# edwinyosorahardjo/compressjs-flattened

Measured on AMD Instinct MI355X. Metric: bzip2 -9 compress MB/s at 1/2/4/8 MI355X; bit-exact output size vs ref, higher is better.
Workload: dtype u32; 1 GPU; Bzip2.compressFile level 9 (899981-byte blocks) on 1 x 100000000 bytes enwik8-shaped synthetic text (tools/textgen.c seed 1), device-resident; per_gpu_bytes=100000000, level=9, parallelism=1 GPU

## Files before the change

### compressjs-flattened_amd/csrc/bwt.hip

```cpp
#include "radix.hpp"
#include <stdlib.h>
#include <string.h>
#include <type_traits>

namespace cjs {

struct Geom { uint32_t nb, stride, n_last; };
__device__ __forceinline__ uint32_t blk_len(const Geom& g, uint32_t blk) { return blk == g.nb - 1 ? g.n_last : g.stride; }
struct VarGeom { uint32_t nb, stride, n_last; const uint32_t* len; };
__device__ __forceinline__ uint32_t blk_len(const VarGeom& g, uint32_t blk) { return g.len[blk]; }

template <typename G>
__global__ __launch_bounds__(256) void bwt_init_keys(const uint8_t* __restrict__ T, G g, int cyclic, int nsym, uint32_t M,
                                                     uint64_t* __restrict__ key, uint32_t* __restrict__ val) {
  for (uint64_t a = (uint64_t)blockIdx.x * 256 + threadIdx.x; a < M; a += (uint64_t)gridDim.x * 256) {
    const uint32_t blk = (uint32_t)(a / g.stride), i = (uint32_t)(a - (uint64_t)blk * g.stride), n = blk_len(g, blk);
    const uint8_t* t = T + (size_t)blk * g.stride;
    uint64_t k = 0;
    if constexpr (std::is_same_v<G, VarGeom>) {
      uint32_t x = i;
      if (i >= n) k = (1ull << (8 * nsym)) | i;
      else for (int j = 0; j < nsym; j++) { k = (k << 8) | t[x]; if (++x == n) x = 0; }
      k |= (uint64_t)blk << (8 * nsym + 1);
    } else if (cyclic) {
// ... 57 lines not shown
    k[it] = key[base + (loc < nvalid ? loc : nvalid - 1u)] >> gshift;
  }
  if (threadIdx.x == 0) sk[0] = base ? key[base - 1] >> gshift : 0;
  if (threadIdx.x == 64) sk[RS_TILE + 1] = base + RS_TILE < A ? key[base + RS_TILE] >> gshift : 0;
#pragma unroll
  for (int it = 0; it < 16; it++) sk[1u + (uint32_t)it * 256 + threadIdx.x] = k[it];
  __syncthreads();
#pragma unroll
  for (int it = 0; it < 16; it++) {
    const uint32_t loc = (uint32_t)it * 256 + threadIdx.x;
    const uint64_t a = base + loc;
    if (loc < nvalid) {
      const bool nh = a == 0 || a == bnd || sk[loc] != k[it];
      const bool nx = a + 1 == A || a + 1 == bnd || sk[loc + 2] != k[it];
      const bool single = nh && nx;
      surv += !single;
      heads += nh && !single;
      if (nh) last = (uint32_t)a + 1u;
    }
    const uint64_t hb = __ballot(loc < nvalid && (base + loc == 0 || base + loc == bnd || sk[loc] != k[it]));
    if (lane_id() == 0) hword[it * 4 + wave_id()] = hb != 0;
  }
  __syncthreads();
  if (threadIdx.x < 8 && base + (threadIdx.x + 1u) * 512u <= A) {
    uint32_t any = 0;
    for (int j = 0; j < 8; j++) any |= hword[threadIdx.x * 8 + j];
    if (!any) atomicOr(big_flag, 1u);
  }
  surv = block_sum<256>(surv, sm);
  heads = block_sum<256>(heads, sm);
  last = wave_max(last);
  if (lane_id() == 0) sm[wave_id()] = last;
  __syncthreads();
  if (threadIdx.x == 0) {
    uint32_t m = sm[0]; for (int i = 1; i < 4; i++) m = sm[i] > m ? sm[i] : m;
    tile_cnt[blockIdx.x] = surv; tile_cnt[T + blockIdx.x] = heads; tile_cnt[2 * (size_t)T + blockIdx.x] = m;
  }
}

constexpr uint32_t HF_NEW = 1u, HF_OLD = 2u;
__device__ __forceinline__ uint32_t hf_bits16(const uint4& v, int bit) {
  const uint32_t M = 0x01020408u;
  const uint32_t n0 = (((v.x >> bit) & 0x01010101u) * M) >> 24, n1 = (((v.y >> bit) & 0x01010101u) * M) >> 24;
  const uint32_t n2 = (((v.z >> bit) & 0x01010101u) * M) >> 24, n3 = (((v.w >> bit) & 0x01010101u) * M) >> 24;
  return (n0 & 15u) | ((n1 & 15u) << 4) | ((n2 & 15u) << 8) | ((n3 & 15u) << 12);
}
__device__ __forceinline__ uint4 hf_load16(const uint8_t* __restrict__ hflag, uint64_t base, uint32_t nvalid, int tid, uint32_t& valid) {
  const uint32_t first = (uint32_t)tid * 16u;
  const uint32_t nv = nvalid > first ? (nvalid - first < 16u ? nvalid - first : 16u) : 0u;
  valid = (1u << nv) - 1u;
  uint4 v = make_uint4(0u, 0u, 0u, 0u);
  if (nv) v = *reinterpret_cast<const uint4*>(hflag + base + first);
  return v;
}
__global__ __launch_bounds__(256) void bwt_key_flags(const uint64_t* __restrict__ key, uint32_t A, uint8_t* __restrict__ hflag) {
  for (uint64_t a = (uint64_t)blockIdx.x * 256 + threadIdx.x; a < A; a += (uint64_t)gridDim.x * 256) {
    const uint64_t k = key[a], p = a ? key[a - 1] : ~k;
    hflag[a] = (uint8_t)((k != p ? HF_NEW : 0u) | ((k >> 20) != (p >> 20) ? HF_OLD : 0u));
  }
}
__global__ __launch_bounds__(256) void bwt_flags_bytes(const uint8_t* __restrict__ hflag, uint32_t A, uint32_t* __restrict__ tile_cnt, uint32_t T,
                                                       uint32_t* __restrict__ big_flag) {
  __shared__ uint32_t nhs[257];
  __shared__ uint32_t sm[4];
  const int tid = threadIdx.x;
  const uint64_t base = (uint64_t)blockIdx.x * RS_TILE;
  const uint32_t nvalid = (uint32_t)((uint64_t)A - base < RS_TILE ? (uint64_t)A - base : RS_TILE);
  uint32_t valid;
  const uint4 v = hf_load16(hflag, base, nvalid, tid, valid);
  const uint32_t nh = hf_bits16(v, 0) & valid;
  nhs[tid] = nh | (~valid & 0xFFFFu);
  if (tid == 0) nhs[256] = base + RS_TILE < A ? (uint32_t)hflag[base + RS_TILE] & HF_NEW : 1u;
  __syncthreads();
  const uint32_t nx = ((nhs[tid] >> 1) | (nhs[tid + 1] << 15)) & 0xFFFFu;
  const uint32_t single = nh & nx;
  uint32_t surv = (uint32_t)__popc(valid & ~single), heads = (uint32_t)__popc(nh & ~single);
  uint32_t last = nh ? (uint32_t)base + (uint32_t)tid * 16u + 32u - (uint32_t)__clz(nh) : 0u;
  {
    const uint64_t any = __ballot(nh != 0);
    const uint32_t run0 = (uint32_t)wave_id() * 2u;
    if (lane_id() == 0) {
      bool bad = false;
      for (uint32_t b = 0; b < 2; b++) bad |= base + (uint64_t)(run0 + b + 1u) * 512u <= A && (uint32_t)(any >> (32 * b)) == 0u;
      if (bad) atomicOr(big_flag, 1u);
    }
  }
  surv = block_sum<256>(surv, sm);
  heads = block_sum<256>(heads, sm);
  last = wave_max(last);
  if (lane_id() == 0) sm[wave_id()] = last;
  __syncthreads();
  if (tid == 0) {
    uint32_t m = sm[0]; for (int i = 1; i < 4; i++) m = sm[i] > m ? sm[i] : m;
    tile_cnt[blockIdx.x] = surv; tile_cnt[T + blockIdx.x] = heads; tile_cnt[2 * (size_t)T + blockIdx.x] = m;
  }
}

__global__ __launch_bounds__(1024) void bwt_scan_tiles(uint32_t* __restrict__ tile_cnt, uint32_t T, uint32_t* __restrict__ counters,
                                                      uint32_t* __restrict__ host_mirror ) {
  __shared__ uint32_t sm[16];
  __shared__ uint32_t mx[1024];
  uint32_t c0 = 0, c1 = 0, cm = 0;
  for (uint32_t base = 0; base < T; base += 1024) {
    const uint32_t i = base + threadIdx.x;
    const bool ok = i < T;
    uint32_t t0, t1;
    const uint32_t v0 = ok ? tile_cnt[i] : 0u, v1 = ok ? tile_cnt[T + i] : 0u, v2 = ok ? tile_cnt[2 * (size_t)T + i] : 0u;
    const uint32_t e0 = block_excl_sum<1024>(v0, sm, t0);
    const uint32_t e1 = block_excl_sum<1024>(v1, sm, t1);
    const uint32_t im = block_incl_max<1024>(v2, sm);
    mx[threadIdx.x] = im;
    __syncthreads();
    const uint32_t prev = threadIdx.x ? mx[threadIdx.x - 1] : 0u;
    const uint32_t chunk_max = mx[1023];
    __syncthreads();
    if (ok) {
      tile_cnt[i] = c0 + e0; tile_cnt[T + i] = c1 + e1;
      tile_cnt[2 * (size_t)T + i] = prev > cm ? prev : cm;
    }
    c0 += t0; c1 += t1; cm = chunk_max > cm ? chunk_max : cm;
  }
  if (threadIdx.x == 0) { counters[0] = c0; counters[1] = c1; host_mirror[0] = c0; host_mirror[1] = c1; host_mirror[4] = counters[4]; counters[4] = 0; }
}

__device__ __forceinline__ uint64_t class_head_before(const uint64_t* __restrict__ key, uint64_t seg0, uint64_t base, int shift, int lane) {
  if (base == seg0) return base;
  const uint64_t target = key[base] >> shift;
  const uint64_t off = base - seg0;
  const uint32_t back = off < 64u ? (uint32_t)off : 64u;
  const bool eq = (uint32_t)lane < back && (key[base - 1u - (uint32_t)lane] >> shift) == target;
  const uint64_t ne = ~__ballot(eq);
  const uint32_t m = ne ? (uint32_t)__builtin_ctzll(ne) : 64u;
  if (m < 64u || off <= 64u) return base - m;
  uint64_t lo = seg0, hi = base - 64u;
  while (hi > lo) {
    const uint64_t len = hi - lo, step = (len + 63u) / 64u, idx = lo + (uint64_t)lane * step;
    const bool hit = idx >= hi || (key[idx] >> shift) == target;
    const uint64_t hits = __ballot(hit);
    const uint32_t j = hits ? (uint32_t)__builtin_ctzll(hits) : 64u;
    if (!j) { hi = lo; break; }
    const uint64_t nhi = lo + (uint64_t)j * step;
    lo += (uint64_t)(j - 1u) * step + 1u;
    if (j < 64u && nhi < hi) hi = nhi;
  }
  return hi;
// ... 81 lines not shown
    const uint32_t first = (uint32_t)lane * 64u;
    const uint32_t nv = nvalid > first ? (nvalid - first < 64u ? nvalid - first : 64u) : 0u;
    const uint64_t vm = nv == 64 ? ~0ull : ((1ull << nv) - 1ull);
    uint64_t ms;
    if constexpr (FIRST) ms = m_sg[lane];
    else {
      const uint64_t mhx = mh | ~vm;
      uint32_t nb = __shfl_down((uint32_t)(mhx & 1ull), 1, 64);
      if (lane == 63) nb = nx_s;
      ms = mh & ((mhx >> 1) | ((uint64_t)nb << 63));
      m_sg[lane] = ms;
    }
    const uint32_t sv = (uint32_t)__popcll(vm & ~ms), hd = (uint32_t)__popcll(mh & ~ms);
    const uint32_t lastrel = mh ? first + 63u - (uint32_t)__builtin_clzll(mh) + 1u : 0u;
    const uint32_t is = wave_incl_sum(sv), ih = wave_incl_sum(hd), im = wave_incl_max(lastrel);
    uint32_t em = __shfl_up(im, 1, 64);
    if (lane == 0) em = 0;
    wp_s[lane] = is - sv; wp_h[lane] = ih - hd; wp_head[lane] = em;
    if (SWEEP == 1 && lane == 63) {
      tile_cnt[tile] = is; tile_cnt[T + tile] = ih; tile_cnt[2 * (size_t)T + tile] = im ? (uint32_t)base + im : 0u;
    }
    if (SWEEP == 1) {
      const uint64_t nz = __ballot(mh != 0);
      bool bad = false;
#pragma unroll
      for (int b = 0; b < 8; b++) bad |= base + (uint64_t)(b + 1) * 512u <= A && ((nz >> (8 * b)) & 0xFFull) == 0;
      if (bad && lane == 0) atomicOr(big_flag, 1u);
    }
  }
  __syncthreads();
  if (SWEEP == 1) carry = carry_s;
  const uint64_t lt = (1ull << lane) - 1ull, le = lane == 63 ? ~0ull : ((2ull << lane) - 1ull);
  uint32_t ub[16];
#pragma unroll
  for (int it = 0; it < 16; it++) ub[it] = 0u;
  const bool emits = U != nullptr && SWEEP != 1;
  if (emits && !carried) {
#pragma unroll
    for (int it = 0; it < 16; it++) {
      const uint32_t e = (uint32_t)it * 256u + tid;
      const bool sing = e < nvalid && ((m_sg[it * 4 + w] >> lane) & 1ull);
      const uint32_t p = FIRST ? (uint32_t)(base + e) : p16[FIRST ? 0 : it];
      const uint32_t vv = (PACKED ? (uint32_t)sk[e + 1] : v16[PACKED ? 0 : it]) & PK_POS_MASK;
      const uint32_t blk = p / g.stride;
      ub[it] = sing ? (uint32_t)Tx[(size_t)blk * g.stride + (vv ? vv - 1u : blk_len(g, blk) - 1u)] : 0u;
    }
  }
#pragma unroll
  for (int it = 0; it < 16; it++) {
    const uint32_t e = (uint32_t)it * 256u + tid;
// ... 14 lines not shown
      }
      const uint32_t p = FIRST ? (uint32_t)a : p16[FIRST ? 0 : it];
      const uint32_t vraw = PACKED ? (uint32_t)sk[e + 1] : v16[PACKED ? 0 : it];
      const uint32_t vv = vraw & PK_POS_MASK;
      const uint32_t pb = PACKED ? (vraw >> PK2_PREV_SHIFT) & 0xFFu : vraw >> VAL_PREV_SHIFT;
      const uint32_t blk = p / g.stride;
      const uint32_t head_pos = p - ((uint32_t)a - head_a);
      if (!keeps_rank && (SWEEP == 0 || (uint32_t)(vv >= hsplit) == half)) R[(size_t)blk * g.stride + vv] = head_pos - blk * g.stride;
      if (SWEEP == 1) continue;
      if ((ms >> lane) & 1ull) {
        if (U) U[p] = (uint8_t)(carried ? pb : ub[it]);
        else __builtin_nontemporal_store(vv, SA + p);
      } else {
        const uint32_t so = sbase + wp_s[wi] + (uint32_t)__popcll(~ms & lt);
        const uint32_t ho = hbase + wp_h[wi] + (uint32_t)__popcll(mh & ~ms & le);
        __builtin_nontemporal_store(carried ? (vv | (pb << VAL_PREV_SHIFT)) : vv, nval + so); __builtin_nontemporal_store(p, npos + so); __builtin_nontemporal_store(ho - 1u, ngord + so);
      }
    }
  }
}

constexpr uint32_t TS_WIN = 4096, TS_MAXGRP = 1024, TS_NOM = TS_WIN - TS_MAXGRP, TS_TINY = 64, TS_GT = 2048;

template <typename G> struct TsGatherT { const uint32_t* R; const uint32_t* pos; const uint32_t* gord; uint32_t h; int cyclic; G g; };
template <bool WMAP> __device__ __forceinline__ uint32_t ts_slot(int s, int tid) {
  return WMAP ? (uint32_t)(tid >> 6) * 1024u + (uint32_t)s * 64u + (uint32_t)(tid & 63) : (uint32_t)s * 256u + (uint32_t)tid;
}
template <bool WMAP, typename TG>
__device__ __forceinline__ uint32_t ts_fused_load(const TG& tg, const uint32_t* __restrict__ val, uint64_t wb, uint32_t L,
                                                  uint32_t (&go)[16], uint32_t (&pv)[16], uint32_t (&pp)[16], uint32_t& gprev) {
  const int tid = threadIdx.x;
#pragma unroll
  for (int s = 0; s < 16; s++) { const uint32_t x = ts_slot<WMAP>(s, tid); go[s] = tg.gord[wb + (x < L ? x : L - 1u)]; }
#pragma unroll
  for (int s = 0; s < 16; s++) { const uint32_t x = ts_slot<WMAP>(s, tid); pv[s] = val[wb + (x < L ? x : L - 1u)]; }
#pragma unroll
  for (int s = 0; s < 16; s++) { const uint32_t x = ts_slot<WMAP>(s, tid); pp[s] = tg.pos[wb + (x < L ? x : L - 1u)]; }
  uint32_t li = 0;
  gprev = 0xFFFFFFFFu;
  if (wb) {
    const uint32_t* q = tg.gord + wb - TS_MAXGRP + (uint32_t)tid * 4u;
    const uint32_t q0 = q[0], q1 = q[1], q2 = q[2], q3 = q[3], g0 = tg.gord[wb];
    gprev = tg.gord[wb - 1];
    li = q3 != g0 ? (uint32_t)tid * 4u + 4u : q2 != g0 ? (uint32_t)tid * 4u + 3u : q1 != g0 ? (uint32_t)tid * 4u + 2u : q0 != g0 ? (uint32_t)tid * 4u + 1u : 0u;
  }
#pragma unroll
// ... 12 lines not shown
__device__ __forceinline__ void ts_fused_gather(const TG& tg, uint32_t need, const uint32_t (&pv)[16], uint32_t (&pp)[16], uint32_t (&rk20)[16]) {
  uint32_t past = 0;
#pragma unroll
  for (int s = 0; s < 16; s++) {
    const uint32_t blk = pp[s] / tg.g.stride, n = blk_len(tg.g, blk);
    uint32_t j = (pv[s] & PK_POS_MASK) + tg.h;
    if (tg.cyclic) { if (j >= n) j %= n; }
    else if (j >= n) { j = 0; past |= 1u << s; }
    pp[s] = blk * tg.g.stride + j;
  }
#pragma unroll
  for (int s = 0; s < 16; s++) rk20[s] = tg.R[((need >> s) & 1u) ? pp[s] : pp[0]];
#pragma unroll
  for (int s = 0; s < 16; s++) rk20[s] = ((past >> s) & 1u) ? 0u : rk20[s] + 1u;
}

__device__ __forceinline__ void ts_ce(uint64_t& a, uint64_t& b, bool up) {
  const bool sw = (a > b) == up;
  const uint64_t x = sw ? b : a, y = sw ? a : b;
  a = x; b = y;
}
template <typename TG>
__global__ __launch_bounds__(256) void bwt_tile_sort(uint64_t* __restrict__ key, uint32_t* __restrict__ val, uint8_t* __restrict__ hflag, uint32_t A,
                                                     uint8_t* __restrict__ dflag, TG tg, uint32_t Tt) {
  __shared__ uint64_t sk[TS_WIN];
  __shared__ uint64_t hm[64];
  __shared__ int32_t wlast[64], wnext[64];
  uint32_t* gk = (uint32_t*)sk;
  const int tid = threadIdx.x, w = tid >> 6, lane = tid & 63;
  __shared__ uint32_t lired[4];
  const uint32_t win = xcd_tile(blockIdx.x, Tt);
  if (win >= Tt) return;
  const uint64_t wb = (uint64_t)win * TS_NOM;
  const uint64_t we = (wb + TS_WIN < A) ? wb + TS_WIN : A;
  const uint32_t L = (uint32_t)(we - wb);
  uint64_t r[16];
  uint32_t pv[16], go[16], pp[16];
  uint32_t gprev;
  {
    const uint32_t li = wave_max(ts_fused_load<false>(tg, val, wb, L, go, pv, pp, gprev));
    if (lane == 0) lired[w] = li;
  }
#pragma unroll
  for (int it = 0; it < 16; it++) gk[(uint32_t)it * 256u + tid] = go[it];
  __syncthreads();
#pragma unroll
  for (int it = 0; it < 16; it++) {
// ... 21 lines not shown
  __shared__ uint32_t mpre[65];
  int any_medium = 0;
  uint32_t hx16[16];
  uint32_t prev_end = 0, needm = 0;
  {
    const uint32_t a01 = lired[0] > lired[1] ? lired[0] : lired[1], a23 = lired[2] > lired[3] ? lired[2] : lired[3];
    prev_end = ts_prev_end(wb, L, we == A, a01 > a23 ? a01 : a23, hm, wnext);
  }
#pragma unroll
  for (int it = 0; it < 16; it++) {
    const uint32_t x = (uint32_t)it * 256u + tid;
    const int wi = it * 4 + w;
    const uint64_t m = hm[wi];
    const uint64_t le = lane == 63 ? ~0ull : ((2ull << lane) - 1ull);
    const uint64_t gt = lane == 63 ? 0ull : ~((2ull << lane) - 1ull);
    int hx = (m & le) ? wi * 64 + 63 - (int)__builtin_clzll(m & le) : wlast[wi];
    int nx = (m & gt) ? wi * 64 + (int)__builtin_ctzll(m & gt) : wnext[wi];
    if (nx > (int)L) nx = (we == A) ? (int)L : (int)TS_WIN + 1;
    const bool valid = x < L;
    const bool small = valid && hx >= 0 && nx <= (int)L && (uint32_t)(nx - hx) <= TS_MAXGRP;
    const bool owned = small && (uint32_t)hx < TS_NOM;
    const bool medium = owned && (nx - hx) > (int)TS_TINY;
    if (owned && dflag) dflag[wb + x] = 0;
    hx16[it] = owned ? ((uint32_t)hx | ((uint32_t)(nx - hx) << 16)) : 0xFFFFFFFFu;
    const uint64_t mb = __ballot(medium);
    if (lane == 0) mm[wi] = mb;
    any_medium |= medium ? 1 : 0;
    needm |= (valid && x >= prev_end && (owned || x < TS_NOM)) ? 1u << it : 0u;
  }
  {
    uint32_t rk20[16];
    ts_fused_gather(tg, needm, pv, pp, rk20);
#pragma unroll
    for (int it = 0; it < 16; it++) {
      const uint32_t x = (uint32_t)it * 256u + tid;
      const bool owned = hx16[it] != 0xFFFFFFFFu;
      if (((needm >> it) & 1u) && !owned) key[wb + x] = ((uint64_t)go[it] << 20) | rk20[it];
      r[it] = owned ? (((uint64_t)(hx16[it] & 0xFFFFu) << 52) | ((uint64_t)rk20[it] << 32) | pv[it])
                    : (((uint64_t)x << 52) | (0xFFFFFull << 32));
    }
  }
  __syncthreads();
  uint32_t* sk32 = reinterpret_cast<uint32_t*>(sk);
#pragma unroll
  for (int it = 0; it < 16; it++) { const uint32_t x = (uint32_t)it * 256u + tid; sk32[x] = ((uint32_t)(r[it] >> 32) << 12) | x; }
  any_medium = __syncthreads_or(any_medium);
// ... 57 lines not shown
      for (uint32_t t = tid; t < (P >> 2); t += 256) {
        const uint32_t i0 = ((t & ~(hj - 1)) << 2) | (t & (hj - 1));
        const bool up = (i0 & kk) == 0;
        uint64_t e0 = sk[i0], e1 = sk[i0 | hj], e2 = sk[i0 | j], e3 = sk[i0 | j | hj];
        ts_ce(e0, e2, up); ts_ce(e1, e3, up); ts_ce(e0, e1, up); ts_ce(e2, e3, up);
        sk[i0] = e0; sk[i0 | hj] = e1; sk[i0 | j] = e2; sk[i0 | j | hj] = e3;
      }
      __syncthreads();
    }
  }
#pragma unroll
  for (int it = 0; it < 16; it++) {
    if (cix[it] != 0xFFFFFFFFu) {
      const uint32_t x = (uint32_t)it * 256u + tid;
      const uint32_t c = cix[it];
      const uint64_t e = sk[c], pe = c ? sk[c - 1] : ~e;
      hflag[wb + x] = (uint8_t)(((e >> 32) != (pe >> 32) ? HF_NEW : 0u) | ((e >> 52) != (pe >> 52) ? HF_OLD : 0u));
      val[wb + x] = (uint32_t)e;
    }
  }
}
template <typename TG>
__global__ __launch_bounds__(256) void bwt_tile_sort_radix(uint64_t* __restrict__ key, uint32_t* __restrict__ val, uint8_t* __restrict__ hflag, uint32_t A,
                                                           uint8_t* __restrict__ dflag, TG tg, uint32_t Tt) {
  __shared__ uint64_t se[TS_WIN];
  __shared__ uint64_t hm[64];
  __shared__ int32_t wlast[64], wnext[64];
  __shared__ uint32_t wcnt[4][256];
  __shared__ uint32_t sm[4];
  uint32_t* gk = (uint32_t*)se;
  const int tid = threadIdx.x, w = tid >> 6, lane = tid & 63;
  __shared__ uint32_t lired[4];
  const uint32_t win = xcd_tile(blockIdx.x, Tt);
  if (win >= Tt) return;
  const uint64_t wb = (uint64_t)win * TS_NOM;
  const uint64_t we = (wb + TS_WIN < A) ? wb + TS_WIN : A;
  const uint32_t L = (uint32_t)(we - wb);
  uint32_t rk20[16], go[16], pv[16], pp[16];
  uint32_t gprev;
  {
    const uint32_t li = wave_max(ts_fused_load<true>(tg, val, wb, L, go, pv, pp, gprev));
    if (lane == 0) lired[w] = li;
#pragma unroll
    for (int s = 0; s < 16; s++) gk[ts_slot<true>(s, tid)] = go[s];
  }
  __syncthreads();
#pragma unroll
// ... 15 lines not shown
    int ir = wave_incl_max(rv);
    int er = __shfl_up(ir, 1, 64); if (lane == 0) er = -((int)TS_WIN + 1);
    const int en = -__shfl(er, 63 - lane, 64);
    wlast[lane] = el; wnext[lane] = en;
  }
  __syncthreads();
  uint32_t prev_end = 0;
  {
    const uint32_t a01 = lired[0] > lired[1] ? lired[0] : lired[1], a23 = lired[2] > lired[3] ? lired[2] : lired[3];
    prev_end = ts_prev_end(wb, L, we == A, a01 > a23 ? a01 : a23, hm, wnext);
  }
  uint32_t comp[16];
  uint32_t ownm = 0, needm = 0;
#pragma unroll
  for (int s = 0; s < 16; s++) {
    const uint32_t x = (uint32_t)w * 1024u + (uint32_t)s * 64u + lane;
    const int wi = w * 16 + s;
    const uint64_t m = hm[wi];
    const uint64_t le = lane == 63 ? ~0ull : ((2ull << lane) - 1ull);
    const uint64_t gt = lane == 63 ? 0ull : ~((2ull << lane) - 1ull);
    const int hx = (m & le) ? wi * 64 + 63 - (int)__builtin_clzll(m & le) : wlast[wi];
    int nx = (m & gt) ? wi * 64 + (int)__builtin_ctzll(m & gt) : wnext[wi];
    if (nx > (int)L) nx = (we == A) ? (int)L : (int)TS_WIN + 1;
    const bool owned = x < L && hx >= 0 && nx <= (int)L && (uint32_t)(nx - hx) <= TS_MAXGRP && (uint32_t)hx < TS_NOM;
    if (owned && dflag) dflag[wb + x] = 0;
    ownm |= owned ? 1u << s : 0u;
    needm |= (x < L && x >= prev_end && (owned || x < TS_NOM)) ? 1u << s : 0u; comp[s] = (uint32_t)hx;
  }
  {
    ts_fused_gather(tg, needm, pv, pp, rk20);
#pragma unroll
    for (int s = 0; s < 16; s++) {
      const uint32_t x = (uint32_t)w * 1024u + (uint32_t)s * 64u + lane;
      const bool owned = (ownm >> s) & 1u;
      if (((needm >> s) & 1u) && !owned) key[wb + x] = ((uint64_t)go[s] << 20) | rk20[s];
      comp[s] = owned ? ((comp[s] << 20) | rk20[s]) : (x << 20);
    }
  }
#pragma unroll
  for (int s = 0; s < 16; s++) if (!((ownm >> s) & 1u)) pv[s] = 0u;
  if (!__syncthreads_or((int)ownm)) return;
#pragma unroll 1
  for (int shift = 0; shift < 32; shift += 8) {
    for (int i = tid; i < 1024; i += 256) (&wcnt[0][0])[i] = 0;
    __syncthreads();
    uint32_t rk[16];
#pragma unroll
    for (int s = 0; s < 16; s++) rk[s] = rank_step((comp[s] >> shift) & 255u, wcnt[w]);
// ... 5 lines not shown
      wcnt[0][tid] = ex; wcnt[1][tid] = ex + c0; wcnt[2][tid] = ex + c0 + c1; wcnt[3][tid] = ex + c0 + c1 + c2;
    }
    __syncthreads();
#pragma unroll
    for (int s = 0; s < 16; s++) {
      const uint32_t d = (comp[s] >> shift) & 255u;
      se[wcnt[w][d] + rk[s]] = ((uint64_t)comp[s] << 32) | pv[s];
    }
    __syncthreads();
#pragma unroll
    for (int s = 0; s < 16; s++) {
      const uint64_t e = se[(uint32_t)w * 1024u + (uint32_t)s * 64u + lane];
      comp[s] = (uint32_t)(e >> 32); pv[s] = (uint32_t)e;
    }
    __syncthreads();
  }
#pragma unroll
  for (int s = 0; s < 16; s++) {
    if ((ownm >> s) & 1u) {
      const uint32_t x = (uint32_t)w * 1024u + (uint32_t)s * 64u + lane;
      const uint32_t pc = x ? (uint32_t)(se[x - 1] >> 32) : ~comp[s];
      hflag[wb + x] = (uint8_t)((comp[s] != pc ? HF_NEW : 0u) | ((comp[s] >> 20) != (pc >> 20) ? HF_OLD : 0u));
      val[wb + x] = pv[s];
    }
  }
}
__global__ __launch_bounds__(1024) void scan_u32_single(uint32_t* __restrict__ arr, uint32_t n, uint32_t* __restrict__ total, uint32_t* __restrict__ host_total) {
  __shared__ uint32_t sm[16];
  uint32_t carry = 0;
  for (uint32_t base = 0; base < n; base += 1024) {
    const uint32_t i = base + threadIdx.x;
    uint32_t v = i < n ? arr[i] : 0u, tot;
    const uint32_t ex = block_excl_sum<1024>(v, sm, tot);
    if (i < n) arr[i] = carry + ex;
    carry += tot;
  }
  if (threadIdx.x == 0) { *total = carry; *host_total = carry; }
}
__device__ __forceinline__ void defer_flags(uint32_t A, const uint8_t* __restrict__ dflag, const uint64_t* __restrict__ key, uint64_t a0,
                                            uint32_t& f, uint32_t& heads, uint64_t (&k8)[8]) {
  f = 0; heads = 0;
  if (a0 >= A) return;
  if (a0 + 8 <= A) {
    const uint64_t w = *(const uint64_t*)(dflag + a0);
#pragma unroll
    for (int j = 0; j < 8; j++) f |= (uint32_t)((w >> (8 * j)) & 1ull) << j;
// ... 155 lines not shown
  for (uint32_t i = threadIdx.x; i < n; i += 256) cnt += r[i] == r0;
  cnt = block_sum<256>(cnt, sm);
  if (threadIdx.x == 0) pidx[blk] = r0 + cnt - 1u;
}

__global__ __launch_bounds__(256) void bwt_emit_sentinel(const uint8_t* __restrict__ T, Geom g, uint32_t M,
                                                         const uint32_t* __restrict__ SA, const uint32_t* __restrict__ R, uint8_t* __restrict__ U, uint32_t Tn) {
  const uint32_t tile = xcd_tile(blockIdx.x, Tn);
  if (tile >= Tn) return;
#pragma unroll 4
  for (int it = 0; it < 16; it++) {
    const uint64_t a = (uint64_t)tile * RS_TILE + (uint32_t)it * 256 + threadIdx.x;
    if (a >= M) break;
    const uint32_t blk = (uint32_t)(a / g.stride), p = (uint32_t)(a - (uint64_t)blk * g.stride), n = blk_len(g, blk);
    const uint8_t* t = T + (size_t)blk * g.stride;
    uint8_t* u = U + (size_t)blk * g.stride;
    const uint32_t s = __builtin_nontemporal_load(SA + a);
    const uint32_t p0 = R[(size_t)blk * g.stride];
    if (p == p0) u[0] = t[n - 1];
    else u[p < p0 ? p + 1 : p] = t[s - 1];
  }
}

enum Counter { CN_SURVIVORS = 0, CN_GROUPS = 1, CN_DEFERRED = 2, CN_DEFERRED_GROUPS = 3, CN_LARGE_GROUP = 4 };

size_t BwtWork::bytes_needed(size_t cap) {
  const size_t T = RadixWork::hist_tiles_for(cap);
  size_t b = 0;
  auto add = [&](size_t n) { b += (n + 255) & ~(size_t)255; };
  add(cap * 8); add(cap * 8); add(cap * 4); add(cap * 4); add(cap * 4); add(cap * 4); add(cap * 4);
  add(cap * 4); add(cap * 4); add(cap); add(cap);
  add(RadixWork::hist_words(T) * 4); add(256 * RadixWork::segs_for(cap) * 4); add(3 * T * 4); add(64);
  return b + 4096;
}
int BwtWork::carve(Arena& a, size_t cap_) {
  cap = cap_;
  const size_t T = RadixWork::hist_tiles_for(cap);
  key[0] = a.take<uint64_t>(cap); key[1] = a.take<uint64_t>(cap);
  val[0] = a.take<uint32_t>(cap); val[1] = a.take<uint32_t>(cap);
  pos[0] = a.take<uint32_t>(cap); pos[1] = a.take<uint32_t>(cap);
  gord = a.take<uint32_t>(cap);
  R = a.take<uint32_t>(cap); SA = a.take<uint32_t>(cap); dflag = a.take<uint8_t>(cap); hflag = a.take<uint8_t>(cap);
  CJS_TRY(rs.carve(a, T, RadixWork::segs_for(cap)));
  tile_cnt = a.take<uint32_t>(3 * T); counters = a.take<uint32_t>(16);
  if (!counters) return CJS_E_OUT_OF_MEMORY;
  if (!h_counters) CJS_HIP_TRY(hipHostMalloc((void**)h_counters.put(), 64));
  if (!ev_scan) CJS_HIP_TRY(hipEventCreateWithFlags(ev_scan.put(), hipEventDisableTiming));
  return 0;
}

struct Plan {
  bool segmented, packed;
  bool sweeps;
  int nsym, bits;
  int gs1, carried;
  SegGeom sg; GenSrc gen;
  const uint8_t* Tx; uint8_t* U;
};
template <typename G>
static Plan plan_round1(const BwtWork& w, const G& g, bool cyclic, const uint8_t* d_T, uint8_t* d_U) {
  constexpr bool VAR = std::is_same_v<G, VarGeom>;
  Plan p;
  const int sym_bits = cyclic ? 8 : 9;
  const uint32_t tps = ((g.nb > 1 ? g.stride : g.n_last) + RS_TILE - 1) / RS_TILE;
  p.segmented = !VAR && (uint64_t)g.nb * tps <= w.rs.hist_tiles && g.nb <= w.rs.bintot_segs && getenv("CJS_NO_SEGMENTED_SORT") == nullptr;
  p.packed = p.segmented && cyclic;
  p.sweeps = g.nb >= 8 && p.packed;
  const int blk_bits = bits_for(g.nb - 1) + (VAR ? 1 : 0);
  p.nsym = p.segmented || (64 - blk_bits) / sym_bits > 7 ? 7 : (64 - blk_bits) / sym_bits;
  p.bits = p.nsym * sym_bits + (p.segmented ? 0 : blk_bits);
  p.gs1 = p.packed ? PK2_GSHIFT : 0;
  p.carried = p.packed ? 1 : 0;
  p.sg = SegGeom{g.nb, g.stride, g.n_last, tps};
  p.gen = GenSrc{d_T, cyclic ? 1 : 0, p.nsym, p.packed ? 2 : 0};
  p.Tx = cyclic ? d_T : nullptr; p.U = cyclic ? d_U : nullptr;
  return p;
}

struct Round {
  int c = 0, pc = 0;
  uint32_t A = 0, h = 0;
  int bits = 0;
  uint32_t ngroups = 0, rounds = 0;
  bool no_large_groups = false;
};

template <typename G>
static int sort_round1(hipStream_t s, BwtWork& w, const G& g, const Plan& p, Round& r, LaunchTimes* lt) {
  if (!p.segmented) {
    const int grid_lin = (int)((r.A + 255) / 256 < 65535u * 16u ? (r.A + 255) / 256 : 65535u * 16u);
    hipLaunchKernelGGL(bwt_init_keys<G>, dim3(grid_lin), dim3(256), 0, s, p.gen.T, g, p.gen.cyclic, p.nsym, r.A, w.key[0], w.val[0]);
    return radix_passes<uint64_t>(s, w.rs, w.key[0], w.val[0], w.key[1], w.val[1], r.c, r.A, 0, r.bits, lt);
  }
  if (!p.packed) return radix_passes<uint64_t>(s, w.rs, w.key[0], w.val[0], w.key[1], w.val[1], r.c, r.A, 0, r.bits, lt, &p.sg, &p.gen);
  CJS_TRY((radix_passes<uint64_t>(s, w.rs, w.key[0], w.val[0], w.key[1], w.val[1], r.c, r.A, PK_KEY_LO, 64, lt, &p.sg, &p.gen, true, false, w.dflag)));
  hipLaunchKernelGGL(bwt_phase2_records, dim3(p.sg.nseg * p.sg.tps), dim3(256), 0, s, w.key[r.c], p.sg, p.gen.T, w.rs.hist, w.key[1 - r.c]);
  r.c = 1 - r.c;
  return radix_passes<uint64_t>(s, w.rs, w.key[0], w.val[0], w.key[1], w.val[1], r.c, r.A, 48, 64, lt, &p.sg, nullptr, true, true, w.dflag);
}

template <typename TG>
static void launch_tile_sort(hipStream_t s, uint32_t Tt, uint64_t* key, uint32_t* val, uint8_t* hflag, uint32_t A, uint8_t* dflag, uint32_t ngroups, const TG& tg) {
  if (ngroups && A / ngroups >= 5) hipLaunchKernelGGL(bwt_tile_sort_radix<TG>, dim3(xcd_grid(Tt)), dim3(256), 0, s, key, val, hflag, A, dflag, tg, Tt);
  else hipLaunchKernelGGL(bwt_tile_sort<TG>, dim3(xcd_grid(Tt)), dim3(256), 0, s, key, val, hflag, A, dflag, tg, Tt);
}
static int sort_round_whole(hipStream_t s, BwtWork& w, Round& r, LaunchTimes* lt) {
  CJS_TRY((radix_passes<uint64_t>(s, w.rs, w.key[0], w.val[0], w.key[1], w.val[1], r.c, r.A, 0, r.bits, lt)));
  hipLaunchKernelGGL(bwt_key_flags, dim3((r.A + 255) / 256 < 8192u ? (r.A + 255) / 256 : 8192u), dim3(256), 0, s, w.key[r.c], r.A, w.hflag);
  CJS_HIP_TRY(hipGetLastError());
  return 0;
}
static bool tile_sorted_round(uint32_t A) { return A >= 2 * TS_WIN; }
template <typename TG>
static int sort_round(hipStream_t s, BwtWork& w, Round& r, LaunchTimes* lt, const TG& tg) {
  if (!tile_sorted_round(r.A)) return sort_round_whole(s, w, r, lt);
  const uint32_t A = r.A, Tt = (A + TS_NOM - 1) / TS_NOM, Tg = (A + TS_GT - 1) / TS_GT;
  const int c = r.c;
  uint8_t* dflag = w.dflag;
  uint32_t* tcount = w.tile_cnt;
  if (r.no_large_groups) {
    launch_tile_sort(s, Tt, w.key[c], w.val[c], w.hflag, A, nullptr, r.ngroups, tg);
    CJS_HIP_TRY(hipGetLastError());
    return 0;
  }
  dev_fill(s, dflag, 1, A);
  launch_tile_sort(s, Tt, w.key[c], w.val[c], w.hflag, A, dflag, r.ngroups, tg);
  uint32_t* hcount = w.rs.hist;
  hipLaunchKernelGGL(bwt_defer_count, dim3(Tg), dim3(256), 0, s, A, dflag, w.key[c], tcount, hcount);
  hipLaunchKernelGGL(scan_u32_single, dim3(1), dim3(1024), 0, s, hcount, Tg, w.counters + CN_DEFERRED_GROUPS, w.h_counters + CN_DEFERRED_GROUPS);
  hipLaunchKernelGGL(scan_u32_single, dim3(1), dim3(1024), 0, s, tcount, Tg, w.counters + CN_DEFERRED, w.h_counters + CN_DEFERRED);
  CJS_HIP_TRY(hipStreamSynchronize(s));
  const uint32_t D = w.h_counters[CN_DEFERRED];
  if (env_debug()) fprintf(stderr, "[cjs bwt]   tile sort: %u of %u suffixes in groups > %u\n", D, A, TS_MAXGRP);
  if (D == 0) { r.no_large_groups = true; return 0; }
  if ((size_t)D > w.cap / 2) {
    const uint32_t Tk = (A + RS_TILE - 1) / RS_TILE;
    hipLaunchKernelGGL(bwt_gather_keys<decltype(tg.g)>, dim3(xcd_grid(Tk)), dim3(256), 0, s, tg.g, tg.cyclic, A, tg.h, tg.R, w.val[c], tg.pos, tg.gord, w.key[c], Tk);
    return sort_round_whole(s, w, r, lt);
  }
  uint64_t* dk0 = w.key[1 - c]; uint64_t* dk1 = dk0 + w.cap / 2;
  uint32_t* dv0 = w.val[1 - c]; uint32_t* dv1 = dv0 + w.cap / 2;
  uint32_t* dpos = w.pos[1 - r.pc];
  hipLaunchKernelGGL(bwt_defer_gather, dim3(Tg), dim3(256), 0, s, w.key[c], w.val[c], A, dflag, tcount, hcount, dk0, dv0, dpos);
  int cur = 0;
  const uint32_t ndg = w.h_counters[CN_DEFERRED_GROUPS];
  CJS_TRY((radix_passes<uint64_t>(s, w.rs, dk0, dv0, dk1, dv1, cur, D, 0, 20 + bits_for(ndg ? ndg - 1 : 0), lt)));
  hipLaunchKernelGGL(bwt_defer_scatter, dim3((D + 255) / 256 < 8192u ? (D + 255) / 256 : 8192u), dim3(256), 0, s, D, cur ? dk1 : dk0, cur ? dv1 : dv0, dpos,
                     w.hflag, w.val[c]);
  CJS_HIP_TRY(hipGetLastError());
// ... 35 lines not shown

template <typename G>
static int bwt_run_impl(hipStream_t s, BwtWork& w, const uint8_t* d_T, const G g, bool cyclic, uint8_t* d_U, uint32_t* d_pidx,
                        cjs_stats* stats, bool resolve_stats) {
  constexpr bool VAR = std::is_same_v<G, VarGeom>;
  const uint32_t nb = g.nb, stride = g.stride, n_last = g.n_last;
  if (nb == 0) return 0;
  if (VAR && (!cyclic || n_last != stride)) return CJS_E_INVALID_ARG;
  const uint64_t M64 = (uint64_t)(nb - 1) * stride + n_last;
  if (M64 > w.cap || M64 >= 0xFFFFF000ull) return CJS_E_INVALID_ARG;
  if (stride > (1u << 20) - 2) return CJS_E_INVALID_ARG;
  const uint32_t M = (uint32_t)M64;
  const uint32_t max_n = nb > 1 ? stride : n_last;
  LaunchTimes& lt = w.lt; lt.reset(); lt.enabled = stats != nullptr; lt.min_elems = M;
  const Plan p = plan_round1(w, g, cyclic, d_T, d_U);
  if (VAR && p.nsym < 3) return CJS_E_INVALID_ARG;

  dev_fill(s, w.counters, 0, 64);
  Round r;
  r.A = M; r.h = (uint32_t)p.nsym; r.bits = p.bits;
  TsGatherT<G> tg{nullptr, nullptr, nullptr, 0u, 0, g};
  for (;;) {
    if (r.rounds == 0) CJS_TRY(sort_round1(s, w, g, p, r, &lt));
    else CJS_TRY(sort_round(s, w, r, &lt, tg));
    CJS_TRY(regroup(s, w, g, p, r));
    CJS_HIP_TRY(hipEventSynchronize(w.ev_scan));
    r.rounds++;
    const uint32_t A2 = w.h_counters[CN_SURVIVORS], NG = w.h_counters[CN_GROUPS];
    if (w.h_counters[CN_LARGE_GROUP] == 0) r.no_large_groups = true;
    if (env_debug()) fprintf(stderr, "[cjs bwt] round %u h=%u A=%u bits=%d -> A'=%u groups=%u\n", r.rounds, r.h, r.A, r.bits, A2, NG);
    r.c = 1 - r.c; r.pc = 1 - r.pc;
    r.A = A2; r.ngroups = NG;
    if (r.A == 0) break;
    if (cyclic && r.h >= max_n) {
      hipLaunchKernelGGL(bwt_flush_active<G>, dim3((r.A + 255) / 256), dim3(256), 0, s, r.A, w.val[r.c], w.pos[r.pc], w.SA, g, p.Tx, p.U, p.carried);
      break;
    }
    if (r.rounds > 40) return CJS_E_HIP;
    prepare_next(s, w, g, cyclic, r, tg);
  }
  hipLaunchKernelGGL(bwt_pidx<G>, dim3(nb), dim3(256), 0, s, g, (int)cyclic, (int)(r.A != 0), w.R, d_pidx);
  if constexpr (!VAR) if (!cyclic) {
    const uint32_t Tn = (M + RS_TILE - 1) / RS_TILE;
    hipLaunchKernelGGL(bwt_emit_sentinel, dim3(xcd_grid(Tn)), dim3(256), 0, s, d_T, g, M, w.SA, w.R, d_U, Tn);
  }
  CJS_HIP_TRY(hipGetLastError());
  if (stats) stats->bwt_rounds = r.rounds;
  if (stats && resolve_stats) {
    CJS_HIP_TRY(hipStreamSynchronize(s));
    lt.resolve(stats);
  }
  return 0;
// ... 14 lines not shown
```

Measured before the change: 9191 MB/s.

## Sort mid-sized BWT groups on chip instead of deferred global path

Records per-tile bitmasks of 512-element runs with no group head, and the scan kernel uses them to detect groups spanning roughly 3.5K+ elements ("huge"). Once no huge groups remain, tile sort appends heads of groups larger than the tile limit to a list. A new kernel then radix-sorts each of those groups (up to 4095 elements) in shared memory. This skips the dflag fill, defer count/scan, host synchronization and global deferred gather/sort for those rounds. It adds an atomic append list and an extra kernel, and depends on the huge-group detection being correct.

```diff
diff --git a/compressjs-flattened_amd/csrc/bwt.hip b/compressjs-flattened_amd/csrc/bwt.hip
--- a/compressjs-flattened_amd/csrc/bwt.hip
+++ b/compressjs-flattened_amd/csrc/bwt.hip
@@ -103,10 +103,17 @@
     if (lane_id() == 0) hword[it * 4 + wave_id()] = hb != 0;
   }
   __syncthreads();
-  if (threadIdx.x < 8 && base + (threadIdx.x + 1u) * 512u <= A) {
-    uint32_t any = 0;
-    for (int j = 0; j < 8; j++) any |= hword[threadIdx.x * 8 + j];
-    if (!any) atomicOr(big_flag, 1u);
+  if (threadIdx.x < 64) {
+    uint32_t any = 1;
+    if (threadIdx.x < 8 && base + (threadIdx.x + 1u) * 512u <= A) {
+      any = 0;
+      for (int j = 0; j < 8; j++) any |= hword[threadIdx.x * 8 + j];
+    }
+    const uint32_t runs = (uint32_t)__ballot(!any) & 0xFFu;
+    if (threadIdx.x == 0) {
+      tile_cnt[3 * (size_t)T + blockIdx.x] = runs;
+      if (runs) atomicOr(big_flag, 1u);
+    }
   }
   surv = block_sum<256>(surv, sm);
   heads = block_sum<256>(heads, sm);
@@ -143,7 +150,7 @@
 __global__ __launch_bounds__(256) void bwt_flags_bytes(const uint8_t* __restrict__ hflag, uint32_t A, uint32_t* __restrict__ tile_cnt, uint32_t T,
                                                        uint32_t* __restrict__ big_flag) {
   __shared__ uint32_t nhs[257];
-  __shared__ uint32_t sm[4];
+  __shared__ uint32_t sm[4], runm[4];
   const int tid = threadIdx.x;
   const uint64_t base = (uint64_t)blockIdx.x * RS_TILE;
   const uint32_t nvalid = (uint32_t)((uint64_t)A - base < RS_TILE ? (uint64_t)A - base : RS_TILE);
@@ -161,9 +168,10 @@
     const uint64_t any = __ballot(nh != 0);
     const uint32_t run0 = (uint32_t)wave_id() * 2u;
     if (lane_id() == 0) {
-      bool bad = false;
-      for (uint32_t b = 0; b < 2; b++) bad |= base + (uint64_t)(run0 + b + 1u) * 512u <= A && (uint32_t)(any >> (32 * b)) == 0u;
-      if (bad) atomicOr(big_flag, 1u);
+      uint32_t runs = 0;
+      for (uint32_t b = 0; b < 2; b++) if (base + (uint64_t)(run0 + b + 1u) * 512u <= A && (uint32_t)(any >> (32 * b)) == 0u) runs |= 1u << (run0 + b);
+      runm[wave_id()] = runs;
+      if (runs) atomicOr(big_flag, 1u);
     }
   }
   surv = block_sum<256>(surv, sm);
@@ -174,6 +182,7 @@
   if (tid == 0) {
     uint32_t m = sm[0]; for (int i = 1; i < 4; i++) m = sm[i] > m ? sm[i] : m;
     tile_cnt[blockIdx.x] = surv; tile_cnt[T + blockIdx.x] = heads; tile_cnt[2 * (size_t)T + blockIdx.x] = m;
+    tile_cnt[3 * (size_t)T + blockIdx.x] = runm[0] | runm[1] | runm[2] | runm[3];
   }
 }
 
@@ -181,12 +190,18 @@
                                                       uint32_t* __restrict__ host_mirror ) {
   __shared__ uint32_t sm[16];
   __shared__ uint32_t mx[1024];
-  uint32_t c0 = 0, c1 = 0, cm = 0;
+  uint32_t c0 = 0, c1 = 0, cm = 0, seven = 0;
   for (uint32_t base = 0; base < T; base += 1024) {
     const uint32_t i = base + threadIdx.x;
     const bool ok = i < T;
     uint32_t t0, t1;
     const uint32_t v0 = ok ? tile_cnt[i] : 0u, v1 = ok ? tile_cnt[T + i] : 0u, v2 = ok ? tile_cnt[2 * (size_t)T + i] : 0u;
+    const uint32_t r0 = ok ? tile_cnt[3 * (size_t)T + i] : 0u, r1 = i + 1 < T ? tile_cnt[3 * (size_t)T + i + 1] : 0u;
+    {
+      const uint32_t m = r0 | (r1 << 8);
+      const uint32_t m2 = m & (m >> 1), m4 = m2 & (m2 >> 2);
+      seven |= m4 & (m4 >> 3) & 0xFFu;
+    }
     const uint32_t e0 = block_excl_sum<1024>(v0, sm, t0);
     const uint32_t e1 = block_excl_sum<1024>(v1, sm, t1);
     const uint32_t im = block_incl_max<1024>(v2, sm);
@@ -201,7 +216,13 @@
     }
     c0 += t0; c1 += t1; cm = chunk_max > cm ? chunk_max : cm;
   }
-  if (threadIdx.x == 0) { counters[0] = c0; counters[1] = c1; host_mirror[0] = c0; host_mirror[1] = c1; host_mirror[4] = counters[4]; counters[4] = 0; }
+  const int huge = __syncthreads_or(seven != 0);
+  if (threadIdx.x == 0) {
+    counters[0] = c0; counters[1] = c1; host_mirror[0] = c0; host_mirror[1] = c1;
+    host_mirror[4] = counters[4]; counters[4] = 0;
+    host_mirror[5] = huge ? 1u : 0u;
+    host_mirror[6] = counters[6]; counters[6] = 0;
+  }
 }
 
 __device__ __forceinline__ uint64_t class_head_before(const uint64_t* __restrict__ key, uint64_t seg0, uint64_t base, int shift, int lane) {
@@ -329,10 +350,13 @@
     }
     if (SWEEP == 1) {
       const uint64_t nz = __ballot(mh != 0);
-      bool bad = false;
-#pragma unroll
-      for (int b = 0; b < 8; b++) bad |= base + (uint64_t)(b + 1) * 512u <= A && ((nz >> (8 * b)) & 0xFFull) == 0;
-      if (bad && lane == 0) atomicOr(big_flag, 1u);
+      uint32_t runs = 0;
+#pragma unroll
+      for (int b = 0; b < 8; b++) if (base + (uint64_t)(b + 1) * 512u <= A && ((nz >> (8 * b)) & 0xFFull) == 0) runs |= 1u << b;
+      if (lane == 0) {
+        tile_cnt[3 * (size_t)T + tile] = runs;
+        if (runs) atomicOr(big_flag, 1u);
+      }
     }
   }
   __syncthreads();
@@ -393,6 +417,8 @@
 
 constexpr uint32_t TS_WIN = 4096, TS_MAXGRP = 1024, TS_NOM = TS_WIN - TS_MAXGRP, TS_TINY = 64, TS_GT = 2048;
 
+struct BigList { uint32_t* heads; uint32_t* count; };
+__device__ __forceinline__ void big_append(const BigList& big, uint32_t head) { big.heads[atomicAdd(big.count, 1u)] = head; }
 template <typename G> struct TsGatherT { const uint32_t* R; const uint32_t* pos; const uint32_t* gord; uint32_t h; int cyclic; G g; };
 template <bool WMAP> __device__ __forceinline__ uint32_t ts_slot(int s, int tid) {
   return WMAP ? (uint32_t)(tid >> 6) * 1024u + (uint32_t)s * 64u + (uint32_t)(tid & 63) : (uint32_t)s * 256u + (uint32_t)tid;
@@ -451,7 +477,7 @@
 }
 template <typename TG>
 __global__ __launch_bounds__(256) void bwt_tile_sort(uint64_t* __restrict__ key, uint32_t* __restrict__ val, uint8_t* __restrict__ hflag, uint32_t A,
-                                                     uint8_t* __restrict__ dflag, TG tg, uint32_t Tt) {
+                                                     uint8_t* __restrict__ dflag, BigList big, TG tg, uint32_t Tt) {
   __shared__ uint64_t sk[TS_WIN];
   __shared__ uint64_t hm[64];
   __shared__ int32_t wlast[64], wnext[64];
@@ -519,6 +545,7 @@
     const bool owned = small && (uint32_t)hx < TS_NOM;
     const bool medium = owned && (nx - hx) > (int)TS_TINY;
     if (owned && dflag) dflag[wb + x] = 0;
+    if (big.heads && valid && hx == (int)x && x < TS_NOM && !small) big_append(big, (uint32_t)(wb + x));
     hx16[it] = owned ? ((uint32_t)hx | ((uint32_t)(nx - hx) << 16)) : 0xFFFFFFFFu;
     const uint64_t mb = __ballot(medium);
     if (lane == 0) mm[wi] = mb;
@@ -622,7 +649,7 @@
 }
 template <typename TG>
 __global__ __launch_bounds__(256) void bwt_tile_sort_radix(uint64_t* __restrict__ key, uint32_t* __restrict__ val, uint8_t* __restrict__ hflag, uint32_t A,
-                                                           uint8_t* __restrict__ dflag, TG tg, uint32_t Tt) {
+                                                           uint8_t* __restrict__ dflag, BigList big, TG tg, uint32_t Tt) {
   __shared__ uint64_t se[TS_WIN];
   __shared__ uint64_t hm[64];
   __shared__ int32_t wlast[64], wnext[64];
@@ -684,8 +711,10 @@
     const int hx = (m & le) ? wi * 64 + 63 - (int)__builtin_clzll(m & le) : wlast[wi];
     int nx = (m & gt) ? wi * 64 + (int)__builtin_ctzll(m & gt) : wnext[wi];
     if (nx > (int)L) nx = (we == A) ? (int)L : (int)TS_WIN + 1;
-    const bool owned = x < L && hx >= 0 && nx <= (int)L && (uint32_t)(nx - hx) <= TS_MAXGRP && (uint32_t)hx < TS_NOM;
+    const bool small = x < L && hx >= 0 && nx <= (int)L && (uint32_t)(nx - hx) <= TS_MAXGRP;
+    const bool owned = small && (uint32_t)hx < TS_NOM;
     if (owned && dflag) dflag[wb + x] = 0;
+    if (big.heads && x < L && hx == (int)x && x < TS_NOM && !small) big_append(big, (uint32_t)(wb + x));
     ownm |= owned ? 1u << s : 0u;
     needm |= (x < L && x >= prev_end && (owned || x < TS_NOM)) ? 1u << s : 0u; comp[s] = (uint32_t)hx;
   }
@@ -737,6 +766,67 @@
       const uint32_t pc = x ? (uint32_t)(se[x - 1] >> 32) : ~comp[s];
       hflag[wb + x] = (uint8_t)((comp[s] != pc ? HF_NEW : 0u) | ((comp[s] >> 20) != (pc >> 20) ? HF_OLD : 0u));
       val[wb + x] = pv[s];
+    }
+  }
+}
+constexpr uint32_t GB_MAX = TS_WIN - 1u, GB_GRID = 1024;
+__global__ __launch_bounds__(256) void bwt_group_sort_big(const uint64_t* __restrict__ key, uint32_t* __restrict__ val, uint8_t* __restrict__ hflag, uint32_t A,
+                                                          const uint32_t* __restrict__ gord, const uint32_t* __restrict__ heads, const uint32_t* __restrict__ count) {
+  __shared__ uint64_t se[TS_WIN];
+  __shared__ uint32_t wcnt[4][256];
+  __shared__ uint32_t sm[4];
+  constexpr uint32_t OUTSIDE = 1u << 20;
+  const int tid = threadIdx.x, w = tid >> 6;
+  const uint32_t ng = *count;
+  for (uint32_t gi = blockIdx.x; gi < ng; gi += gridDim.x) {
+    const uint32_t head = heads[gi];
+    const uint32_t lim = A - head < GB_MAX ? A - head : GB_MAX;
+    const uint32_t g0 = gord[head];
+    uint32_t comp[16], pv[16], go[16];
+#pragma unroll
+    for (int s = 0; s < 16; s++) { const uint32_t x = ts_slot<true>(s, tid); go[s] = gord[head + (x < lim ? x : 0u)]; }
+#pragma unroll
+    for (int s = 0; s < 16; s++) { const uint32_t x = ts_slot<true>(s, tid); comp[s] = (uint32_t)key[head + (x < lim ? x : 0u)] & 0xFFFFFu; }
+#pragma unroll
+    for (int s = 0; s < 16; s++) { const uint32_t x = ts_slot<true>(s, tid); pv[s] = val[head + (x < lim ? x : 0u)]; }
+#pragma unroll
+    for (int s = 0; s < 16; s++) if (ts_slot<true>(s, tid) >= lim || go[s] != g0) { comp[s] = OUTSIDE; pv[s] = 0u; }
+#pragma unroll 1
+    for (int shift = 0; shift < 24; shift += 8) {
+      for (int i = tid; i < 1024; i += 256) (&wcnt[0][0])[i] = 0;
+      __syncthreads();
+      uint32_t rk[16];
+#pragma unroll
+      for (int s = 0; s < 16; s++) rk[s] = rank_step((comp[s] >> shift) & 255u, wcnt[w]);
+      __syncthreads();
+      {
+        const uint32_t c0 = wcnt[0][tid], c1 = wcnt[1][tid], c2 = wcnt[2][tid], c3 = wcnt[3][tid];
+        uint32_t total;
+        const uint32_t ex = block_excl_sum<256>(c0 + c1 + c2 + c3, sm, total);
+        wcnt[0][tid] = ex; wcnt[1][tid] = ex + c0; wcnt[2][tid] = ex + c0 + c1; wcnt[3][tid] = ex + c0 + c1 + c2;
+      }
+      __syncthreads();
+#pragma unroll
+      for (int s = 0; s < 16; s++) {
+        const uint32_t d = (comp[s] >> shift) & 255u;
+        se[wcnt[w][d] + rk[s]] = ((uint64_t)comp[s] << 32) | pv[s];
+      }
+      __syncthreads();
+#pragma unroll
+      for (int s = 0; s < 16; s++) {
+        const uint64_t e = se[ts_slot<true>(s, tid)];
+        comp[s] = (uint32_t)(e >> 32); pv[s] = (uint32_t)e;
+      }
+      __syncthreads();
+    }
+#pragma unroll
+    for (int s = 0; s < 16; s++) {
+      const uint32_t x = ts_slot<true>(s, tid);
+      if (comp[s] != OUTSIDE) {
+        const uint32_t pc = x ? (uint32_t)(se[x - 1] >> 32) : ~comp[s];
+        hflag[head + x] = (uint8_t)((comp[s] != pc ? HF_NEW : 0u) | (x ? 0u : HF_OLD));
+        val[head + x] = pv[s];
+      }
     }
   }
 }
@@ -938,7 +1028,7 @@
   }
 }
 
-enum Counter { CN_SURVIVORS = 0, CN_GROUPS = 1, CN_DEFERRED = 2, CN_DEFERRED_GROUPS = 3, CN_LARGE_GROUP = 4 };
+enum Counter { CN_SURVIVORS = 0, CN_GROUPS = 1, CN_DEFERRED = 2, CN_DEFERRED_GROUPS = 3, CN_LARGE_GROUP = 4, CN_HUGE_GROUP = 5, CN_BIG_GROUPS = 6 };
 
 size_t BwtWork::bytes_needed(size_t cap) {
   const size_t T = RadixWork::hist_tiles_for(cap);
@@ -946,7 +1036,7 @@
   auto add = [&](size_t n) { b += (n + 255) & ~(size_t)255; };
   add(cap * 8); add(cap * 8); add(cap * 4); add(cap * 4); add(cap * 4); add(cap * 4); add(cap * 4);
   add(cap * 4); add(cap * 4); add(cap); add(cap);
-  add(RadixWork::hist_words(T) * 4); add(256 * RadixWork::segs_for(cap) * 4); add(3 * T * 4); add(64);
+  add(RadixWork::hist_words(T) * 4); add(256 * RadixWork::segs_for(cap) * 4); add(4 * T * 4); add(64);
   return b + 4096;
 }
 int BwtWork::carve(Arena& a, size_t cap_) {
@@ -958,7 +1048,7 @@
   gord = a.take<uint32_t>(cap);
   R = a.take<uint32_t>(cap); SA = a.take<uint32_t>(cap); dflag = a.take<uint8_t>(cap); hflag = a.take<uint8_t>(cap);
   CJS_TRY(rs.carve(a, T, RadixWork::segs_for(cap)));
-  tile_cnt = a.take<uint32_t>(3 * T); counters = a.take<uint32_t>(16);
+  tile_cnt = a.take<uint32_t>(4 * T); counters = a.take<uint32_t>(16);
   if (!counters) return CJS_E_OUT_OF_MEMORY;
   if (!h_counters) CJS_HIP_TRY(hipHostMalloc((void**)h_counters.put(), 64));
   if (!ev_scan) CJS_HIP_TRY(hipEventCreateWithFlags(ev_scan.put(), hipEventDisableTiming));
@@ -999,6 +1089,8 @@
   int bits = 0;
   uint32_t ngroups = 0, rounds = 0;
   bool no_large_groups = false;
+  bool no_huge_groups = false;
+  bool on_chip = false;
 };
 
 template <typename G>
@@ -1016,9 +1108,9 @@
 }
 
 template <typename TG>
-static void launch_tile_sort(hipStream_t s, uint32_t Tt, uint64_t* key, uint32_t* val, uint8_t* hflag, uint32_t A, uint8_t* dflag, uint32_t ngroups, const TG& tg) {
-  if (ngroups && A / ngroups >= 5) hipLaunchKernelGGL(bwt_tile_sort_radix<TG>, dim3(xcd_grid(Tt)), dim3(256), 0, s, key, val, hflag, A, dflag, tg, Tt);
-  else hipLaunchKernelGGL(bwt_tile_sort<TG>, dim3(xcd_grid(Tt)), dim3(256), 0, s, key, val, hflag, A, dflag, tg, Tt);
+static void launch_tile_sort(hipStream_t s, uint32_t Tt, uint64_t* key, uint32_t* val, uint8_t* hflag, uint32_t A, uint8_t* dflag, BigList big, uint32_t ngroups, const TG& tg) {
+  if (ngroups && A / ngroups >= 5) hipLaunchKernelGGL(bwt_tile_sort_radix<TG>, dim3(xcd_grid(Tt)), dim3(256), 0, s, key, val, hflag, A, dflag, big, tg, Tt);
+  else hipLaunchKernelGGL(bwt_tile_sort<TG>, dim3(xcd_grid(Tt)), dim3(256), 0, s, key, val, hflag, A, dflag, big, tg, Tt);
 }
 static int sort_round_whole(hipStream_t s, BwtWork& w, Round& r, LaunchTimes* lt) {
   CJS_TRY((radix_passes<uint64_t>(s, w.rs, w.key[0], w.val[0], w.key[1], w.val[1], r.c, r.A, 0, r.bits, lt)));
@@ -1035,12 +1127,21 @@
   uint8_t* dflag = w.dflag;
   uint32_t* tcount = w.tile_cnt;
   if (r.no_large_groups) {
-    launch_tile_sort(s, Tt, w.key[c], w.val[c], w.hflag, A, nullptr, r.ngroups, tg);
+    launch_tile_sort(s, Tt, w.key[c], w.val[c], w.hflag, A, nullptr, BigList{nullptr, nullptr}, r.ngroups, tg);
     CJS_HIP_TRY(hipGetLastError());
     return 0;
   }
+  if (r.no_huge_groups) {
+    const BigList big{w.pos[1 - r.pc], w.counters + CN_BIG_GROUPS};
+    launch_tile_sort(s, Tt, w.key[c], w.val[c], w.hflag, A, nullptr, big, r.ngroups, tg);
+    const uint32_t most = A / (TS_MAXGRP + 1u) + 1u;
+    hipLaunchKernelGGL(bwt_group_sort_big, dim3(most < GB_GRID ? most : GB_GRID), dim3(256), 0, s, w.key[c], w.val[c], w.hflag, A, tg.gord, big.heads, big.count);
+    CJS_HIP_TRY(hipGetLastError());
+    r.on_chip = true;
+    return 0;
+  }
   dev_fill(s, dflag, 1, A);
-  launch_tile_sort(s, Tt, w.key[c], w.val[c], w.hflag, A, dflag, r.ngroups, tg);
+  launch_tile_sort(s, Tt, w.key[c], w.val[c], w.hflag, A, dflag, BigList{nullptr, nullptr}, r.ngroups, tg);
   uint32_t* hcount = w.rs.hist;
   hipLaunchKernelGGL(bwt_defer_count, dim3(Tg), dim3(256), 0, s, A, dflag, w.key[c], tcount, hcount);
   hipLaunchKernelGGL(scan_u32_single, dim3(1), dim3(1024), 0, s, hcount, Tg, w.counters + CN_DEFERRED_GROUPS, w.h_counters + CN_DEFERRED_GROUPS);
@@ -1122,12 +1223,18 @@
   TsGatherT<G> tg{nullptr, nullptr, nullptr, 0u, 0, g};
   for (;;) {
     if (r.rounds == 0) CJS_TRY(sort_round1(s, w, g, p, r, &lt));
-    else CJS_TRY(sort_round(s, w, r, &lt, tg));
+    else { r.on_chip = false; CJS_TRY(sort_round(s, w, r, &lt, tg)); }
     CJS_TRY(regroup(s, w, g, p, r));
     CJS_HIP_TRY(hipEventSynchronize(w.ev_scan));
     r.rounds++;
     const uint32_t A2 = w.h_counters[CN_SURVIVORS], NG = w.h_counters[CN_GROUPS];
+    if (r.on_chip) {
+      const uint32_t nbig = w.h_counters[CN_BIG_GROUPS];
+      if (env_debug()) fprintf(stderr, "[cjs bwt]   big groups: %u groups of %u..%u suffixes sorted on chip\n", nbig, TS_MAXGRP + 1u, GB_MAX);
+      if (nbig == 0) r.no_large_groups = true;
+    }
     if (w.h_counters[CN_LARGE_GROUP] == 0) r.no_large_groups = true;
+    if (w.h_counters[CN_HUGE_GROUP] == 0) r.no_huge_groups = true;
     if (env_debug()) fprintf(stderr, "[cjs bwt] round %u h=%u A=%u bits=%d -> A'=%u groups=%u\n", r.rounds, r.h, r.A, r.bits, A2, NG);
     r.c = 1 - r.c; r.pc = 1 - r.pc;
     r.A = A2; r.ngroups = NG;
```

Measured after the change: 9397 MB/s (median of 6 runs). 2.2% higher.
